# tudelft-iv/CCVPE

Hardware: AMD Instinct MI355X
Metric: image-pairs/sec (higher is better)
Workload: dtype f32

## Files before the change

ccvpe_amd/_lib.py:

```python
import ctypes
import os
import subprocess

import torch

_HERE = os.path.dirname(os.path.abspath(__file__))
LIB_PATH = os.environ.get("CCVPE_LIB") or os.path.join(_HERE, "libccvpe_hip.so")
CSRC_DIR = os.path.join(_HERE, "csrc")

c_float_p = ctypes.c_void_p
c_int = ctypes.c_int
c_float = ctypes.c_float
c_void_p = ctypes.c_void_p


class ConvDesc(ctypes.Structure):
    _fields_ = [
        ("src0", c_void_p), ("src1", c_void_p), ("gate", c_void_p), ("w", c_void_p),
        ("scale", c_void_p), ("shift", c_void_p), ("residual", c_void_p), ("dst", c_void_p),
        ("c0", c_int), ("ld0", c_int), ("c1", c_int), ("ld1", c_int),
        ("batch", c_int), ("in_h", c_int), ("in_w", c_int),
        ("kh", c_int), ("kw", c_int), ("stride", c_int), ("pad", c_int),
        ("n", c_int), ("kpad", c_int), ("ldd", c_int), ("ldres", c_int),
        ("act", c_int), ("out_mode", c_int),
# ... 60 lines not shown
    "ccvpe_upconv3x3_s3_form_ok": (c_int, [ctypes.POINTER(UpconvDesc), c_int]),
    "ccvpe_upconv3x3_s3_route": (c_int, [ctypes.POINTER(UpconvDesc), c_int]),
    "ccvpe_upconv3x3_s3_form_f32": (c_int, [ctypes.POINTER(UpconvDesc), c_int, c_void_p]),
    "ccvpe_set_s3_quad": (c_int, [c_int]),
    "ccvpe_pw_s3_ok": (c_int, [ctypes.POINTER(ConvDesc)]),
    "ccvpe_pw_s3_route": (c_int, [ctypes.POINTER(ConvDesc)]),
    "ccvpe_pw_s3_f32": (c_int, [ctypes.POINTER(ConvDesc), c_void_p]),
    "ccvpe_stem_conv_f32": (c_int, [c_void_p] * 5 + [c_int] * 4 + [c_void_p]),
    "ccvpe_dwconv_nblk": (c_int, [c_int] * 4),
    "ccvpe_dwconv_f32": (c_int, [c_void_p] * 6 + [c_int] * 7 + [c_void_p]),
    "ccvpe_mbconv_front_nblk": (c_int, [c_int] * 6),
    "ccvpe_stem_dw_nblk": (c_int, [c_int] * 3),
    "ccvpe_stem_dw_f32": (c_int, [c_void_p] * 9 + [c_int] * 4 + [c_void_p]),
    "ccvpe_stem_dw_bf16": (c_int, [c_void_p] * 9 + [c_int] * 4 + [c_void_p]),
    "ccvpe_mbconv_front_f32": (c_int, [c_void_p, c_void_p, c_int] + [c_void_p] * 7 + [c_int] * 8 + [c_void_p]),
    "ccvpe_se_gate_f32": (c_int, [c_void_p, c_int, c_float] + [c_void_p] * 5 + [c_int] * 3 + [c_void_p]),
    "ccvpe_ground_descriptor_f32": (c_int, [c_void_p, c_int, c_void_p, c_void_p, ctypes.POINTER(c_int),
                                            c_void_p, c_int, c_int, c_int, c_void_p]),
    "ccvpe_match_level_f32": (c_int, [c_void_p, c_int, c_void_p, c_int, c_int, ctypes.POINTER(c_int),
                                      c_int, c_int, c_int, c_int, c_int, c_void_p, c_void_p, c_int, c_int,
                                      c_int, c_int, c_void_p]),
    "ccvpe_head_conv3x3_f32": (c_int, [c_void_p] * 4 + [c_int] * 5 + [c_void_p]),
    "ccvpe_cast_bf16_f32": (c_int, [c_void_p, c_void_p, ctypes.c_long, c_void_p]),
    "ccvpe_softmax_rows_f32": (c_int, [c_void_p, c_void_p, c_int, c_int, c_void_p]),
    "ccvpe_eval_postprocess_f32": (c_int, [c_void_p, c_void_p, c_void_p, c_int, c_int, c_int, c_void_p]),
    "ccvpe_eval_metrics_f32": (c_int, [c_void_p] * 7 + [c_int, c_int, c_int, c_void_p]),
    "ccvpe_infonce_scratch_floats": (c_int, [c_int, c_int]),
    "ccvpe_infonce_loss_f32": (c_int, [c_void_p, c_void_p, c_float, c_void_p, c_void_p, c_void_p, c_int, c_int, c_void_p]),
    "ccvpe_cross_entropy_loss_f32": (c_int, [c_void_p] * 4 + [c_int, c_int, c_void_p]),
    "ccvpe_orientation_loss_f32": (c_int, [c_void_p] * 5 + [c_int, c_int, c_void_p]),
# ... 132 lines not shown
```

ccvpe_amd/csrc/mbconv_front.hip:

```cpp
#include "common.h"
#include "mbconv_plane.h"
#include <type_traits>

namespace ccvpe {

typedef float f32x4 __attribute__((ext_vector_type(4)));
typedef int mbf_i32x4 __attribute__((ext_vector_type(4)));
__device__ __forceinline__ f32x4 keepv(f32x4 v, bool keep) {
  return __builtin_bit_cast(f32x4, __builtin_bit_cast(mbf_i32x4, v) & (keep ? -1 : 0));
}

struct MbFrontParams {
  const void* x;
  const void* w_exp;
  const float* s0;
  const float* b0;
  const float* w_dw;
  const float* s1;
  const float* b1;
  void* y;
  float* se_partial;
  int H, W, Cin, kpad, mid, Ho, Wo, circular;
  int tiles_x, tiles_y, nchunks, total_blocks;
  int ngroups, cpg;
// ... 157 lines not shown
    for (int o = 4; o < 64; o <<= 1) {
#pragma unroll
      for (int r = 0; r < 4; ++r) sum[r] += __shfl_xor(sum[r], o, 64);
    }
    if (lane < 4) *reinterpret_cast<f32x4*>(red + (wave * 4 + lane) * 4) = sum;
    __syncthreads();
    if (tid < 4) {
      f32x4 t = *reinterpret_cast<const f32x4*>(red + tid * 4);
#pragma unroll
      for (int w = 1; w < 4; ++w) t += *reinterpret_cast<const f32x4*>(red + (w * 4 + tid) * 4);
      *reinterpret_cast<f32x4*>(p.se_partial + ((size_t)b * (p.tiles_x * p.tiles_y) + ty * p.tiles_x + tx) * p.mid + c0 + tid * 4) = t;
    }
  }
}

static int mbf_toh(int k, int stride, int cin) {
  const int n = (cin + 15) / 16;
  if (stride == 2) return n == 1 ? 8 : 4;
  return (n == 1 && k == 3) ? 16 : 8;
}

static bool mbf_supported(int W, int cin, int mid, int k, int sk = 16, int stride = -1) {
  (void)W;
  if (k == 5 && stride == 2 && cin > 32) return false;
  return cin % 8 == 0 && cin <= 16 * MBF_MAX_KK && cin <= sk * MBF_MAX_KK && mid % 16 == 0;
}

}

using namespace ccvpe;
// ... 8 lines not shown
  return ((Ho + toh - 1) / toh) * ((Wo + 15) / 16);
}

extern "C" int ccvpe_mbconv_front_route(int in_h, int in_w, int cin, int mid, int k, int stride, int is_bf16, int batch) {
  if (!(k == 3 || k == 5) || !(stride == 1 || stride == 2)) return CCVPE_EINVAL;
  if (mbf_supported(in_w, cin, mid, k, 16, stride)) return 1;
  if (!(g_mbplane_mode & 1) || mbplane_nblk(in_h, in_w, cin, mid, k, stride) <= 0) return 0;
  return (is_bf16 && (g_mbplane_mode & 4) && mbband_takes(in_h, in_w, cin, mid, k, stride, batch)) ? 3 : 2;
}

extern "C" int ccvpe_mbconv_band_plan(int in_h, int in_w, int cin, int mid, int k, int stride, int batch) {
  if (ccvpe_mbconv_front_route(in_h, in_w, cin, mid, k, stride, 1, batch) != 3) return 0;
  return mbband_plan_packed(in_h, in_w, cin, mid, k, stride, batch);
}

template <typename TE>
static int mbconv_front_any(const void* x, const void* w_exp, int kpad, const float* s0, const float* b0,
                            const float* w_dw, const float* s1, const float* b1, void* y, float* se_partial, int B,
                            int H, int W, int cin, int mid, int k, int stride, int circular, void* stream) {
  constexpr int SK = 4 * (16 / (int)sizeof(TE));
  if (!(k == 3 || k == 5) || !(stride == 1 || stride == 2)) return fail(CCVPE_EINVAL, "mbconv_front: k/stride unsupported");
  if (!mbf_supported(W, cin, mid, k, 16, stride) && (g_mbplane_mode & 1) && mbplane_nblk(H, W, cin, mid, k, stride) > 0)
    return mbplane_launch(sizeof(TE) == 2, 1, x, w_exp, kpad, s0, b0, w_dw, s1, b1, y, se_partial, B, H, W, cin, mid, k, stride,
                          circular, stream);
  if (!mbf_supported(W, cin, mid, k, SK, stride)) return fail(CCVPE_EINVAL, "mbconv_front: shape not supported (W=%d cin=%d mid=%d)", W, cin, mid);
  if (kpad % SK || kpad < cin) return fail(CCVPE_EINVAL, "mbconv_front: bad kpad");
  if (!aligned16(x) || !aligned16(w_exp) || !aligned16(s0) || !aligned16(b0) || !aligned16(s1) || !aligned16(b1) ||
      !aligned16(y) || !aligned16(se_partial) || !aligned16(w_dw))
    return fail(CCVPE_EINVAL, "mbconv_front: pointers must be 16-byte aligned");
  if ((double)H * W * cin * sizeof(TE) >= 4294967296.0) return fail(CCVPE_EINVAL, "mbconv_front: sample larger than 4 GB");
  if (circular && W < k) return fail(CCVPE_EINVAL, "mbconv_front: W too small for circular wrap");
  MbFrontParams p;
  p.x = x; p.w_exp = w_exp; p.s0 = s0; p.b0 = b0; p.w_dw = w_dw; p.s1 = s1; p.b1 = b1; p.y = y; p.se_partial = se_partial;
  p.H = H; p.W = W; p.Cin = cin; p.kpad = kpad; p.mid = mid; p.circular = circular;
  const int total_pad = (stride == 1) ? (k - 1) : (k - 2);
  p.Ho = (H + total_pad - k) / stride + 1;
  p.Wo = (W + total_pad - k) / stride + 1;
  const int toh = mbf_toh(k, stride, cin);
  p.tiles_x = (p.Wo + 15) / 16;
  p.tiles_y = (p.Ho + toh - 1) / toh;
  p.nchunks = mid / 16;
  const long tiles = (long)p.tiles_x * p.tiles_y * B;
  int ng = (int)((2048 + tiles - 1) / tiles);
  if (ng > p.nchunks) ng = p.nchunks;
  if (ng < 1) ng = 1;
  p.cpg = (p.nchunks + ng - 1) / ng;
  p.ngroups = (p.nchunks + p.cpg - 1) / p.cpg;
  const long total = tiles * p.ngroups;
  if (total > 0x7fffffffL) return fail(CCVPE_EINVAL, "mbconv_front: grid too large");
  p.total_blocks = (int)total;
  hipStream_t st = (hipStream_t)stream;
  const int nkk = (cin + SK - 1) / SK;
  int rc = CCVPE_OK;
  auto go = [&](auto kern, int lds_floats) {
    const int lds = lds_floats * 4;
    static DevCache lds_set;
    if ((rc = ensure_dyn_lds(lds_set, kern, lds, "mbconv_front"))) return;
    hipLaunchKernelGGL(kern, dim3(p.total_blocks), dim3(256), lds, st, p);
  };
#define MBF_N(K_, S_, TOH_)                                                                                  \
  if (nkk == 1) go(mbconv_front_kernel<TE, K_, S_, 1, TOH_>, MbfGeom<K_, S_, TOH_>::LDS_FLOATS);                \
  else if (nkk == 2) go(mbconv_front_kernel<TE, K_, S_, 2, TOH_>, MbfGeom<K_, S_, TOH_>::LDS_FLOATS);           \
  else go(mbconv_front_kernel<TE, K_, S_, 3, TOH_>, MbfGeom<K_, S_, TOH_>::LDS_FLOATS)
#define MBF_T(K_, S_, BIG_, SMALL_)                                                                          \
  if (toh == BIG_) { go(mbconv_front_kernel<TE, K_, S_, 1, BIG_>, MbfGeom<K_, S_, BIG_>::LDS_FLOATS); } else { MBF_N(K_, S_, SMALL_); }
// ... 11 lines not shown

extern "C" int ccvpe_mbconv_front_f32(const float* x, const float* w_exp, int kpad, const float* s0, const float* b0,
                                      const float* w_dw, const float* s1, const float* b1, float* y,
                                      float* se_partial, int B, int H, int W, int cin, int mid, int k, int stride,
                                      int circular, void* stream) {
  return mbconv_front_any<float>(x, w_exp, kpad, s0, b0, w_dw, s1, b1, y, se_partial, B, H, W, cin, mid, k, stride,
                                 circular, stream);
}
extern "C" int ccvpe_mbconv_front_bf16(const void* x, const void* w_exp, int kpad, const float* s0, const float* b0,
                                       const float* w_dw, const float* s1, const float* b1, void* y,
                                       float* se_partial, int B, int H, int W, int cin, int mid, int k, int stride,
                                       int circular, void* stream) {
  return mbconv_front_any<cc_bf16>(x, w_exp, kpad, s0, b0, w_dw, s1, b1, y, se_partial, B, H, W, cin, mid, k, stride,
                                   circular, stream);
}
```

ccvpe_amd/csrc/plan.hip:

```cpp
#include <cstring>
#include <string>
#include <unordered_map>
#include <utility>
#include <vector>

#include "common.h"

namespace ccvpe {

enum : uint32_t { K_INT = 0, K_FLT = 1, K_NULL = 2, K_WEIGHTS = 3, K_WORKSPACE = 4, K_GRD = 5, K_SAT = 6, K_STREAM = 7, K_BLOB = 8 };

template <typename A> struct FromSlot {
  static A get(uint64_t v) { return (A)(int64_t)v; }
};
template <typename P> struct FromSlot<P*> {
  static P* get(uint64_t v) { return reinterpret_cast<P*>((uintptr_t)v); }
};
template <> struct FromSlot<float> {
  static float get(uint64_t v) { uint32_t b = (uint32_t)v; float f; std::memcpy(&f, &b, 4); return f; }
};
template <typename... A, size_t... I>
static int invoke_seq(int (*f)(A...), const uint64_t* v, std::index_sequence<I...>) { return f(FromSlot<A>::get(v[I])...); }
template <typename... A>
static int invoke(int (*f)(A...), const uint64_t* v, int n) {
  if (n != (int)sizeof...(A)) return fail(CCVPE_EINVAL, "plan: call has %d arguments, the entry point takes %d", n, (int)sizeof...(A));
  return invoke_seq(f, v, std::index_sequence_for<A...>{});
}
typedef int (*Invoker)(const uint64_t*, int);

#define CCVPE_REG(fn) {#fn, [](const uint64_t* v, int n) -> int { return invoke(fn, v, n); }}
static const std::unordered_map<std::string, Invoker>& registry() {
  static const std::unordered_map<std::string, Invoker> r = {
      CCVPE_REG(ccvpe_conv_igemm_f32), CCVPE_REG(ccvpe_conv_igemm_bf16), CCVPE_REG(ccvpe_conv_igemm_splitk_f32),
      CCVPE_REG(ccvpe_conv_igemm_splitk_bf16), CCVPE_REG(ccvpe_conv3x3_match1_bf16), CCVPE_REG(ccvpe_conv3x3_wino_f32),
      CCVPE_REG(ccvpe_upconv3x3_f32), CCVPE_REG(ccvpe_upconv3x3_bf16), CCVPE_REG(ccvpe_upconv3x3_s3_f32), CCVPE_REG(ccvpe_pw_s3_f32),
      CCVPE_REG(ccvpe_tail512_f32), CCVPE_REG(ccvpe_tail512_bf16), CCVPE_REG(ccvpe_stem_conv_f32), CCVPE_REG(ccvpe_stem_conv_bf16),
      CCVPE_REG(ccvpe_stem_dw_f32), CCVPE_REG(ccvpe_stem_dw_bf16),
      CCVPE_REG(ccvpe_dwconv_f32), CCVPE_REG(ccvpe_dwconv_bf16), CCVPE_REG(ccvpe_mbconv_front_f32), CCVPE_REG(ccvpe_mbconv_front_bf16),
      CCVPE_REG(ccvpe_se_gate_f32), CCVPE_REG(ccvpe_ground_descriptor_f32), CCVPE_REG(ccvpe_match_level_f32),
      CCVPE_REG(ccvpe_match_level_bf16), CCVPE_REG(ccvpe_head_conv3x3_f32), CCVPE_REG(ccvpe_head_conv3x3_bf16),
      CCVPE_REG(ccvpe_softmax_rows_f32), CCVPE_REG(ccvpe_softmax_apply_f32), CCVPE_REG(ccvpe_cast_bf16_f32), CCVPE_REG(ccvpe_eval_postprocess_f32),
  };
  return r;
}
#undef CCVPE_REG

struct Patch { uint32_t call, arg, kind; uint64_t off; };
struct BlobPatch { uint32_t blob, field, kind; uint64_t off; };
struct Call { Invoker fn; std::string name; uint32_t first, nargs, sid; int wait_on; };
struct Output { uint64_t off, bytes; uint32_t dtype, ndim; long long dims[4], strides[4]; };

}

// ... 241 lines not shown
```

ccvpe_amd/models.py:

```python
import torch
import torch.nn as nn

from . import ops
from .synth import B0_BLOCKS, MODEL_SPECS, state_dict_spec

BN_EPS = 1e-3
SKIP_BLOCKS = (15, 10, 4, 2, 0)
MATCH_STRIDES = {"vigor": (64, 32, 16, 8, 4, 2),
                 "kitti": (128, 64, 32, 16, 8, 8),
                 "oxford": (64, 32, 16, 8, 4, 2)}


def window_offset(kind, channels, length):
    return int(channels / 2 - length / 2) if kind == "oxford" else 0


def _round_up(v, m):
    return (v + m - 1) // m * m


class _Holder(nn.Module):

    def forward(self, *a, **k):
        raise RuntimeError("parameter holder is not callable; use the owning CVM_* module")
# ... 59 lines not shown
def _pack_pw_s3(w):
    if w is None or w.dtype != torch.float32 or w.dim() != 2 or w.shape[1] % 16 or w.shape[0] % 16:
        return None
    npad, k = w.shape
    return torch.cat(_split3_bf16(w.reshape(npad, k // 16, 16).permute(1, 0, 2)), -1).contiguous()


def _unpack_pw_s3(w3):
    nst, npad, _ = w3.shape
    return tuple(w3[..., 16 * q:16 * q + 16].float().permute(1, 0, 2).reshape(npad, nst * 16) for q in range(3))


PW_S3_MIN_MID = 240


def _pack_encoder(sd, p, dtype=torch.float32, fold_bn=True, s3=False):
    fold = _fold_bn if fold_bn else (lambda _sd, _p: (None, None))
    e = _Obj()
    e.stem_w = sd[p + "._conv_stem.weight"].permute(2, 3, 1, 0).contiguous()
    e.stem_scale, e.stem_shift = fold(sd, p + "._bn0")
    e.blocks = []
    for i, (k, s, ex, cin, cout) in enumerate(B0_BLOCKS):
        b = _Obj()
        bp = "%s._blocks.%d" % (p, i)
        b.k, b.s, b.expand, b.cin, b.cout, b.mid = k, s, ex != 1, cin, cout, cin * ex
        if b.expand:
            b.w_exp = _pack_conv(sd[bp + "._expand_conv.weight"], dtype)
            b.s0, b.b0 = fold(sd, bp + "._bn0")
        b.w_dw = sd[bp + "._depthwise_conv.weight"].reshape(b.mid, k, k).permute(1, 2, 0).contiguous()
        b.s1, b.b1 = fold(sd, bp + "._bn1")
        b.se_w1 = sd[bp + "._se_reduce.weight"].reshape(-1, b.mid).contiguous()
        b.se_b1 = sd[bp + "._se_reduce.bias"].contiguous()
        b.se_w2 = sd[bp + "._se_expand.weight"].reshape(b.mid, -1).t().contiguous()
        b.se_b2 = sd[bp + "._se_expand.bias"].contiguous()
        b.w_proj = _pack_conv(sd[bp + "._project_conv.weight"], dtype)
        b.w_proj3 = _pack_pw_s3(b.w_proj) if s3 and b.mid >= PW_S3_MIN_MID else None
        b.s2, b.b2 = fold(sd, bp + "._bn2")
        b.skip = (s == 1 and cin == cout)
        e.blocks.append(b)
    e.w_head = _pack_conv(sd[p + "._conv_head.weight"], dtype)
    e.w_head3 = _pack_pw_s3(e.w_head) if s3 else None
    e.head_scale, e.head_shift = fold(sd, p + "._bn1")
    return e
# ... 16 lines not shown
OVERLAP_DECODERS_MAX_BATCH = 128


def _overlap_decoders(precision, batch=1):
    return _OVERLAP_ENV == "1" or (_OVERLAP_ENV == "auto" and precision == "bf16" and batch <= OVERLAP_DECODERS_MAX_BATCH)
FOLD_LEVELS = tuple(int(c) for c in __import__("os").environ.get("CCVPE_FOLD_LEVELS", "012345"))
FOLD_MIN_PIXELS = int(__import__("os").environ.get("CCVPE_FOLD_MIN_PIXELS", "2048"))
FUSE_TAIL = __import__("os").environ.get("CCVPE_FUSE_TAIL", "1") != "0"
SPLIT_TAIL = __import__("os").environ.get("CCVPE_SPLIT_TAIL", "1") != "0"
WINO = __import__("os").environ.get("CCVPE_WINO", "1") != "0"
SPLIT3 = __import__("os").environ.get("CCVPE_SPLIT3", "1") != "0"
SPLIT3_TAIL = SPLIT3 and __import__("os").environ.get("CCVPE_SPLIT3_TAIL", "1") != "0"
SPLIT3_MIN_OK = 2
SPLIT3_PW = SPLIT3 and __import__("os").environ.get("CCVPE_SPLIT3_PW", "1") != "0"
SPLIT3_PW_MIN_OK = 2
PACK_GRAPH = __import__("os").environ.get("CCVPE_PACK_GRAPH", "1") != "0"
PACK_GATHER = __import__("os").environ.get("CCVPE_PACK_GATHER", "1") != "0"
FUSE_MATCH = __import__("os").environ.get("CCVPE_FUSE_MATCH", "1") != "0"
FUSE_STEM = __import__("os").environ.get("CCVPE_FUSE_STEM", "1") != "0"
EVAL_TWO_STREAMS = __import__("os").environ.get("CCVPE_EVAL_TWO_STREAMS", "1") != "0"


def _tail_split(precision, x, cout):
    if x.dtype != torch.float32:
        return 0
    if precision == "bf16":
        return 1 if SPLIT_TAIL and cout == 1 else 0
    return 2 if SPLIT3 and SPLIT3_TAIL else 0


# ... 206 lines not shown

def _run_encoder(e, img, circular, multiscale, dtype=torch.float32):
    blk0 = e.blocks[0]
    stem_fused = (FUSE_STEM and not blk0.expand and blk0.k == 3 and blk0.s == 1 and blk0.mid == 32
                  and ops.stem_dw_supported(img.shape[2], img.shape[3], circular) > 0)
    x = None if stem_fused else ops.stem_conv(img, e.stem_w, e.stem_scale, e.stem_shift, circular, out_dtype=dtype)
    feats = []
    for blk in e.blocks:
        if x is not None:
            b, h, w, _ = x.shape
        if x is None:
            u, part = ops.stem_dw(img, e.stem_w, e.stem_scale, e.stem_shift, blk.w_dw, blk.s1, blk.b1, circular,
                                  out_dtype=dtype)
            b = u.shape[0]
        elif blk.expand and ops.mbconv_front_supported(h, w, blk.cin, blk.mid, blk.k, blk.s):
            u, part = ops.mbconv_front(x, blk.w_exp, blk.s0, blk.b0, blk.w_dw, blk.s1, blk.b1, blk.mid,
                                       blk.k, blk.s, circular)
        else:
            t = x
            if blk.expand:
                t = ops.conv_igemm(x, blk.cin, blk.w_exp, blk.mid, batch=b, in_h=h, in_w=w,
                                   scale=blk.s0, shift=blk.b0, act=ops.ACT_SWISH)
            u, part = ops.dwconv(t, blk.w_dw, blk.s1, blk.b1, blk.k, blk.s, circular)
        ho, wo = u.shape[1], u.shape[2]
        gate = ops.se_gate(part, ho * wo, blk.se_w1, blk.se_b1, blk.se_w2, blk.se_b2)
        x = _pw(u, blk.mid, blk.w_proj, getattr(blk, "w_proj3", None), blk.cout, batch=b, in_h=ho, in_w=wo, gate=gate,
                scale=blk.s2, shift=blk.b2, residual=x if blk.skip else None)
        if multiscale:
            feats.append(x)
    b, h, w, _ = x.shape
    f = _pw(x, 320, e.w_head, getattr(e, "w_head3", None), 1280, batch=b, in_h=h, in_w=w, scale=e.head_scale,
            shift=e.head_shift, act=ops.ACT_SWISH)
# ... 324 lines not shown
```

ccvpe_amd/ops.py:

```python
import ctypes

import torch

from . import _lib
from ._lib import ConvDesc, check

ACT_NONE, ACT_RELU, ACT_SWISH, ACT_RELU_MASK = 0, 1, 2, 3
SPLIT_K_CALLS = 0
SPLIT_K = __import__("os").environ.get("CCVPE_SPLIT_K", "1") == "1"
OUT_NHWC, OUT_DECONV2X = 0, 1

_recorder = None


def set_recorder(rec):
    global _recorder
    _recorder = rec


class LaunchRecorder(object):

    def __init__(self):
        self.items = []

# ... 531 lines not shown
    part = _empty((b, nblk, mid), device=x.device, dtype=torch.float32)
    rec = _recorder
    ev0 = rec.begin() if rec is not None else None
    fn = lib.ccvpe_mbconv_front_f32 if dt == torch.float32 else lib.ccvpe_mbconv_front_bf16
    check(fn(_ptr(x), _ptr(w_exp), w_exp.shape[1], _ptr(s0), _ptr(b0), _ptr(w_dw), _ptr(s1), _ptr(b1), _ptr(y),
             _ptr(part), b, h, wd, cin, mid, k, stride, int(bool(circular)), _stream()), "ccvpe_mbconv_front")
    if rec is not None:
        flops = 2.0 * b * h * wd * cin * mid + 2.0 * b * ho * wo * mid * k * k
        nbytes = (4.0 if dt == torch.float32 else 2.0) * (b * h * wd * cin + b * ho * wo * mid)
        route = lib.ccvpe_mbconv_front_route(h, wd, cin, mid, k, stride, int(dt != torch.float32), b)
        kname = {1: "mbconv_front_kernel", 2: "mbconv_plane_kernel", 3: "mbconv_band_kernel"}.get(route, "mbconv_front_kernel")
        rec.end("%s<%d,%d>" % (kname, k, stride), "in %dx%dx%d mid %d" % (h, wd, cin, mid), flops, nbytes, ev0)
    return y, part


def se_gate(part, hw, w1, b1, w2, b2):
    lib = _lib.load()
    for t, nm in ((part, "part"), (w1, "w1"), (b1, "b1"), (w2, "w2"), (b2, "b2")):
        _chk(t, nm)
    b, nblk, c = part.shape
    cs = w1.shape[0]
    gate = _empty((b, c), device=part.device, dtype=torch.float32)
    check(lib.ccvpe_se_gate_f32(_ptr(part), nblk, 1.0 / float(hw), _ptr(w1), _ptr(b1), _ptr(w2), _ptr(b2),
                                _ptr(gate), b, c, cs, _stream()), "ccvpe_se_gate_f32")
    return gate


def ground_descriptor(y1, wh, bh, cd):
    lib = _lib.load()
    for t, nm in ((y1, "y1"), (wh, "wh"), (bh, "bh")):
# ... 231 lines not shown
```

ccvpe_amd/plan.py:

```python
import ctypes
import struct
import weakref

import torch

from . import _lib, ops

K_INT, K_FLT, K_NULL, K_WEIGHTS, K_WORKSPACE, K_GRD, K_SAT, K_STREAM, K_BLOB = range(9)
ALIGN = 256

LAUNCHES = ("ccvpe_conv_igemm_f32", "ccvpe_conv_igemm_bf16", "ccvpe_conv_igemm_splitk_f32", "ccvpe_conv_igemm_splitk_bf16",
            "ccvpe_conv3x3_match1_bf16", "ccvpe_conv3x3_wino_f32",
            "ccvpe_upconv3x3_f32", "ccvpe_upconv3x3_bf16", "ccvpe_upconv3x3_s3_f32", "ccvpe_pw_s3_f32", "ccvpe_tail512_f32", "ccvpe_tail512_bf16", "ccvpe_stem_conv_f32",
            "ccvpe_stem_conv_bf16", "ccvpe_stem_dw_f32", "ccvpe_stem_dw_bf16", "ccvpe_dwconv_f32", "ccvpe_dwconv_bf16", "ccvpe_mbconv_front_f32", "ccvpe_mbconv_front_bf16",
            "ccvpe_se_gate_f32", "ccvpe_ground_descriptor_f32", "ccvpe_match_level_f32", "ccvpe_match_level_bf16",
            "ccvpe_head_conv3x3_f32", "ccvpe_head_conv3x3_bf16", "ccvpe_softmax_rows_f32", "ccvpe_softmax_apply_f32", "ccvpe_cast_bf16_f32",
            "ccvpe_eval_postprocess_f32")
QUERIES = ("ccvpe_tail512_partials", "ccvpe_conv3x3_match1_ok", "ccvpe_conv3x3_wino_ok", "ccvpe_upconv3x3_s3_ok", "ccvpe_conv_igemm_splitk_floats", "ccvpe_conv_igemm_route", "ccvpe_conv3x3_variant", "ccvpe_upconv3x3_route", "ccvpe_upconv3x3_s3_route", "ccvpe_pw_s3_ok", "ccvpe_pw_s3_route", "ccvpe_dwconv_nblk", "ccvpe_mbconv_front_nblk", "ccvpe_mbconv_front_route", "ccvpe_mbconv_band_plan", "ccvpe_stem_dw_nblk",
           "ccvpe_last_error", "ccvpe_abi_version")


class _Arena(object):

    def __init__(self, size):
        self.size, self.free, self.peak = size, [(0, size)], 0

    def alloc(self, nbytes):
        n = max(ALIGN, (nbytes + ALIGN - 1) // ALIGN * ALIGN)
        for i, (off, sz) in enumerate(self.free):
            if sz >= n:
                if sz == n:
                    del self.free[i]
                else:
# ... 338 lines not shown
```

include/ccvpe_hip.h:

```cpp
#ifndef CCVPE_HIP_H
#define CCVPE_HIP_H

#ifdef __cplusplus
extern "C" {
#endif

#define CCVPE_OK 0
#define CCVPE_EINVAL (-1)
#define CCVPE_ELAUNCH (-2)

#define CCVPE_ACT_NONE 0
#define CCVPE_ACT_RELU 1
#define CCVPE_ACT_SWISH 2
#define CCVPE_ACT_RELU_MASK 3

#define CCVPE_OUT_NHWC 0
#define CCVPE_OUT_DECONV2X 1

#define CCVPE_MAX_SHIFTS 48

const char* ccvpe_last_error(void);
int ccvpe_abi_version(void);

typedef struct ccvpe_conv_desc {
// ... 106 lines not shown
int ccvpe_stem_dw_nblk(int in_h, int in_w, int circular);
int ccvpe_stem_dw_f32(const float* x_nchw, const float* w, const float* s0, const float* b0, const float* w_dw,
                      const float* s1, const float* b1, float* y, float* se_partial, int batch, int in_h,
                      int in_w, int circular, void* stream);
int ccvpe_stem_dw_bf16(const float* x_nchw, const float* w, const float* s0, const float* b0, const float* w_dw,
                       const float* s1, const float* b1, void* y, float* se_partial, int batch, int in_h,
                       int in_w, int circular, void* stream);

int ccvpe_mbconv_front_nblk(int in_h, int in_w, int cin, int mid, int k, int stride);
int ccvpe_mbconv_front_route(int in_h, int in_w, int cin, int mid, int k, int stride, int is_bf16, int batch);
int ccvpe_mbconv_band_plan(int in_h, int in_w, int cin, int mid, int k, int stride, int batch);
int ccvpe_mbconv_front_f32(const float* x, const float* w_exp, int kpad, const float* s0, const float* b0,
                           const float* w_dw, const float* s1, const float* b1, float* y, float* se_partial,
                           int batch, int in_h, int in_w, int cin, int mid, int k, int stride, int circular,
                           void* stream);

int ccvpe_se_gate_f32(const float* se_partial, int nblk, float inv_hw, const float* w1, const float* b1,
                      const float* w2, const float* b2, float* gate, int batch, int channels,
                      int squeezed, void* stream);

int ccvpe_ground_descriptor_f32(const float* y1, int ld, const float* wh, const float* bh, const int* cd,
                                float* out, int batch, int h, int w, void* stream);

int ccvpe_set_match_mfma(int on);
#define CCVPE_MATCH_ROUTE_INTS 10
int ccvpe_match_route(int elem_size, int L, const int* shifts, int n_shifts, int n_max, int n_tail, int stride,
                      int window_offset, int ldx, int ldo, int batch, int hw, int channels, int* out);
int ccvpe_match_level_f32(const float* x, int ldx, const float* g, int ldg, int L, const int* shifts,
                          int n_shifts, int n_max, int n_tail, int stride, int window_offset, float* scores,
                          float* dstx, int ldo, int batch, int hw, int channels, void* stream);
// ... 175 lines not shown
```

Baseline: 2856.

## Add split-bf16 three-plane MFMA path for fused MBConv expand+depthwise front

Adds a new fused MBConv front kernel for f32 inputs. It splits each activation into three bf16 planes and runs the expand 1x1 conv as bf16 MFMA chains against pre-packed three-plane weights, then feeds a depthwise conv, swish and SE partial sums. The aim is to replace the f32 expand GEMM with bf16 matrix-core work while keeping near-f32 accuracy. Weights are double-buffered in LDS across channel chunks, and the path is gated by a per-shape tile-count threshold. In exchange it uses more LDS and registers, and its result can differ slightly from pure f32.

```diff
diff --git a/ccvpe_amd/_lib.py b/ccvpe_amd/_lib.py
--- a/ccvpe_amd/_lib.py
+++ b/ccvpe_amd/_lib.py
@@ -98,6 +98,8 @@
     "ccvpe_stem_dw_f32": (c_int, [c_void_p] * 9 + [c_int] * 4 + [c_void_p]),
     "ccvpe_stem_dw_bf16": (c_int, [c_void_p] * 9 + [c_int] * 4 + [c_void_p]),
     "ccvpe_mbconv_front_f32": (c_int, [c_void_p, c_void_p, c_int] + [c_void_p] * 7 + [c_int] * 8 + [c_void_p]),
+    "ccvpe_mbconv_front_s3_ok": (c_int, [c_int] * 7),
+    "ccvpe_mbconv_front_s3_f32": (c_int, [c_void_p, c_void_p, c_int] + [c_void_p] * 7 + [c_int] * 8 + [c_void_p]),
     "ccvpe_se_gate_f32": (c_int, [c_void_p, c_int, c_float] + [c_void_p] * 5 + [c_int] * 3 + [c_void_p]),
     "ccvpe_ground_descriptor_f32": (c_int, [c_void_p, c_int, c_void_p, c_void_p, ctypes.POINTER(c_int),
                                             c_void_p, c_int, c_int, c_int, c_void_p]),
diff --git a/ccvpe_amd/csrc/mbconv_front.hip b/ccvpe_amd/csrc/mbconv_front.hip
--- a/ccvpe_amd/csrc/mbconv_front.hip
+++ b/ccvpe_amd/csrc/mbconv_front.hip
@@ -1,5 +1,6 @@
 #include "common.h"
 #include "mbconv_plane.h"
+#include "split3_impl.h"
 #include <type_traits>
 
 namespace ccvpe {
@@ -195,6 +196,218 @@
   }
 }
 
+typedef unsigned mbf_u32x4 __attribute__((ext_vector_type(4)));
+
+template <int K, int S, int NKB, int TOH>
+struct Mbf3Geom {
+  using G = MbfGeom<K, S, TOH>;
+  static constexpr int W_DW = NKB * 16 * S3_ROW;
+  static constexpr int W_OFF = G::LDS_FLOATS;
+  static constexpr int LDS_FLOATS = W_OFF + 2 * W_DW;
+};
+
+template <int K, int S, int NKB, int TOH, int WGS>
+__global__ __launch_bounds__(256, WGS) void mbconv_front_s3_kernel(const MbFrontParams p) {
+  using G = MbfGeom<K, S, TOH>;
+  using G3 = Mbf3Geom<K, S, NKB, TOH>;
+  constexpr int PB = (S == 1) ? (K - 1) / 2 : (K - 2) / 2;
+  constexpr int IW = G::IW, NPX = G::NPX, NT = G::NT, TPW = G::TPW, PITCH = G::PITCH;
+  constexpr int KYU = 1;
+  constexpr int W_DW = G3::W_DW, WPIECES = W_DW / 4, WPT = (WPIECES + 255) / 256;
+  extern __shared__ __attribute__((aligned(16))) float sm[];
+  float* tile = sm;
+  float* wdw = sm + NT * 16 * PITCH;
+  float* red = wdw + 2 * K * K * 16;
+  float* wl = sm + G3::W_OFF;
+
+  const int tid = threadIdx.x;
+  const int lane = tid & 63;
+  const int wave = tid >> 6;
+  const int g4 = lane >> 4;
+
+  int lb;
+  {
+    const int q = p.total_blocks / 8, r = p.total_blocks % 8;
+    const int xcd = blockIdx.x % 8, loc = blockIdx.x / 8;
+    lb = (xcd < r ? xcd * (q + 1) : r * (q + 1) + (xcd - r) * q) + loc;
+  }
+  const int grp = lb % p.ngroups;
+  lb /= p.ngroups;
+  const int tx = lb % p.tiles_x;
+  const int ty = (lb / p.tiles_x) % p.tiles_y;
+  const int b = lb / (p.tiles_x * p.tiles_y);
+  const int oy0 = ty * TOH, ox0 = tx * 16;
+  const int iy0 = oy0 * S - PB, ix0 = ox0 * S - PB;
+  const int q4 = g4 * 4;
+
+  f32x4 sc0, sh0, sc1, sh1, wdr, wr[WPT];
+  const int cg = tid & 3;
+  auto load_chunk_params = [&](int chunk) {
+    const int c0 = chunk * 16;
+#pragma unroll
+    for (int j = 0; j < WPT; ++j) {
+      const int idx = tid + 256 * j;
+      if (idx < WPIECES) {
+        const int kb = idx / 96, pc = idx - kb * 96;
+        wr[j] = *reinterpret_cast<const f32x4*>(reinterpret_cast<const float*>(p.w_exp) + ((size_t)kb * p.mid + c0) * S3_ROW + pc * 4);
+      }
+    }
+    sc0 = *reinterpret_cast<const f32x4*>(p.s0 + c0 + q4);
+    sh0 = *reinterpret_cast<const f32x4*>(p.b0 + c0 + q4);
+    sc1 = *reinterpret_cast<const f32x4*>(p.s1 + c0 + cg * 4);
+    sh1 = *reinterpret_cast<const f32x4*>(p.b1 + c0 + cg * 4);
+    const int wi = tid < K * K * 4 ? tid : 0;
+    wdr = *reinterpret_cast<const f32x4*>(p.w_dw + (size_t)(wi >> 2) * p.mid + c0 + (wi & 3) * 4);
+  };
+  auto park_w = [&](int chunk) {
+#pragma unroll
+    for (int j = 0; j < WPT; ++j) {
+      const int idx = tid + 256 * j;
+      if (idx < WPIECES) *reinterpret_cast<f32x4*>(wl + (chunk & 1) * W_DW + idx * 4) = wr[j];
+    }
+  };
+  const int chunk_begin = grp * p.cpg, chunk_end = min(p.nchunks, chunk_begin + p.cpg);
+  load_chunk_params(chunk_begin);
+
+  const float* xb = reinterpret_cast<const float*>(p.x) + (size_t)b * p.H * p.W * p.Cin;
+  mbf_u32x4 xa1[TPW][NKB], xa2[TPW][NKB];
+  unsigned pvalid = 0;
+#pragma unroll
+  for (int i = 0; i < TPW; ++i) {
+    const int q = 16 * (wave + 4 * i) + (lane & 15);
+    const int hy = q / IW, hx = q - hy * IW;
+    const int gy = iy0 + hy;
+    int gx = ix0 + hx;
+    if (p.circular) gx = gx < 0 ? gx + p.W : (gx >= p.W ? gx - p.W : gx);
+    const bool ok = q < NPX && (unsigned)gy < (unsigned)p.H && (unsigned)gx < (unsigned)p.W;
+    pvalid |= ok ? (1u << i) : 0u;
+    const unsigned off = ok ? (unsigned)((gy * p.W + gx) * p.Cin) * 4u : 0u;
+#pragma unroll
+    for (int kb = 0; kb < NKB; ++kb) {
+      const int ch = kb * 16 + (g4 & 1) * 8;
+      const char* src = reinterpret_cast<const char*>(xb) + off + (unsigned)(ch < p.Cin ? ch : 0) * 4u;
+      const f32x4 v0 = *reinterpret_cast<const f32x4*>(src), v1 = *reinterpret_cast<const f32x4*>(src + 16);
+      u32x2 h0, m0, l0, h1, m1, l1;
+      split3(v0, h0, m0, l0);
+      split3(v1, h1, m1, l1);
+      const mbf_u32x4 hi = {h0[0], h0[1], h1[0], h1[1]}, mi = {m0[0], m0[1], m1[0], m1[1]}, lo = {l0[0], l0[1], l1[0], l1[1]};
+      xa1[i][kb] = g4 < 2 ? hi : mi;
+      xa2[i][kb] = g4 < 2 ? lo : hi;
+    }
+  }
+  park_w(chunk_begin);
+  __syncthreads();
+
+  constexpr int NOUT = G::NOUT;
+  constexpr int NCOLS = (NOUT - 1) * S + K;
+  constexpr int XG = 16 / NOUT;
+  const int oxg = (tid >> 2) % XG;
+  const int oyl = (tid >> 2) / XG;
+  const int oy = oy0 + oyl;
+  const int oxl = oxg * NOUT;
+  const bool row_ok = oy < p.Ho;
+  float* yrow = reinterpret_cast<float*>(p.y) + ((size_t)(b * p.Ho + (row_ok ? oy : 0)) * p.Wo) * p.mid;
+  const float* trow = tile + ((oyl * S) * IW + oxl * S) * PITCH + cg * 4;
+  const S3Frag fr(g4);
+
+  for (int chunk = chunk_begin; chunk < chunk_end; ++chunk) {
+    const int c0 = chunk * 16;
+    float* wd = wdw + (chunk & 1) * K * K * 16;
+    if (tid < K * K * 4) *reinterpret_cast<f32x4*>(wd + tid * 4) = wdr;
+    cc_bf16x8 w1[NKB], w2[NKB], w3[NKB];
+    {
+      const float* wrow = wl + (chunk & 1) * W_DW + (lane & 15) * S3_ROW;
+#pragma unroll
+      for (int kb = 0; kb < NKB; ++kb) {
+        w1[kb] = __builtin_bit_cast(cc_bf16x8, *reinterpret_cast<const f32x4*>(wrow + kb * 16 * S3_ROW + fr.w1));
+        w2[kb] = __builtin_bit_cast(cc_bf16x8, *reinterpret_cast<const f32x4*>(wrow + kb * 16 * S3_ROW + fr.w2));
+        w3[kb] = __builtin_bit_cast(cc_bf16x8, *reinterpret_cast<const f32x4*>(wrow + kb * 16 * S3_ROW + fr.w3));
+      }
+    }
+    auto has = [&](int i) { return i < TPW - 1 || wave + 4 * i < NT; };
+    auto chain = [&](int i) {
+      f32x4 acc = {0.f, 0.f, 0.f, 0.f};
+#pragma unroll
+      for (int kb = 0; kb < NKB; ++kb) {
+        const cc_bf16x8 a1 = __builtin_bit_cast(cc_bf16x8, xa1[i][kb]), a2 = __builtin_bit_cast(cc_bf16x8, xa2[i][kb]);
+        acc = __builtin_amdgcn_mfma_f32_16x16x32_bf16(w1[kb], a1, acc, 0, 0, 0);
+        acc = __builtin_amdgcn_mfma_f32_16x16x32_bf16(w2[kb], a1, acc, 0, 0, 0);
+        acc = __builtin_amdgcn_mfma_f32_16x16x32_bf16(w3[kb], a2, acc, 0, 0, 0);
+      }
+      return acc;
+    };
+    auto finish = [&](int i, f32x4 acc) {
+      f32x4 o;
+#pragma unroll
+      for (int r = 0; r < 4; ++r) o[r] = swishf(acc[r] * sc0[r] + sh0[r]);
+      const bool inside = (pvalid >> i) & 1u;
+#pragma unroll
+      for (int r = 0; r < 4; ++r) o[r] = inside ? o[r] : 0.f;
+      *reinterpret_cast<f32x4*>(tile + (16 * (wave + 4 * i) + (lane & 15)) * PITCH + q4) = o;
+    };
+    constexpr int NPAIR = (TPW + 1) / 2;
+    f32x4 pacc[2][2];
+    pacc[0][0] = chain(0);
+    if (1 < TPW && has(1)) pacc[0][1] = chain(1);
+    __builtin_amdgcn_sched_barrier(0);
+#pragma unroll
+    for (int pp = 0; pp < NPAIR; ++pp) {
+      const int n0 = 2 * pp + 2, n1 = 2 * pp + 3;
+      if (n0 < TPW && has(n0)) pacc[(pp + 1) & 1][0] = chain(n0);
+      if (n1 < TPW && has(n1)) pacc[(pp + 1) & 1][1] = chain(n1);
+      if (has(2 * pp)) finish(2 * pp, pacc[pp & 1][0]);
+      if (2 * pp + 1 < TPW && has(2 * pp + 1)) finish(2 * pp + 1, pacc[pp & 1][1]);
+      __builtin_amdgcn_sched_barrier(0);
+    }
+    const f32x4 sc1c = sc1, sh1c = sh1;
+    __syncthreads();
+    const bool more = chunk + 1 < chunk_end;
+    if (more) load_chunk_params(chunk + 1);
+
+    f32x4 acc[NOUT];
+#pragma unroll
+    for (int t = 0; t < NOUT; ++t) acc[t] = (f32x4){0.f, 0.f, 0.f, 0.f};
+#pragma unroll KYU
+    for (int ky = 0; ky < K; ++ky) {
+      f32x4 col[NCOLS];
+#pragma unroll
+      for (int j = 0; j < NCOLS; ++j) col[j] = *reinterpret_cast<const f32x4*>(trow + (ky * IW + j) * PITCH);
+#pragma unroll
+      for (int kx = 0; kx < K; ++kx) {
+        const f32x4 wv = *reinterpret_cast<const f32x4*>(wd + (ky * K + kx) * 16 + cg * 4);
+#pragma unroll
+        for (int t = 0; t < NOUT; ++t) acc[t] += col[t * S + kx] * wv;
+      }
+    }
+    f32x4 sum = {0.f, 0.f, 0.f, 0.f};
+#pragma unroll
+    for (int t = 0; t < NOUT; ++t) {
+      const int ox = ox0 + oxl + t;
+      f32x4 o = acc[t] * sc1c + sh1c;
+#pragma unroll
+      for (int r = 0; r < 4; ++r) o[r] = swishf(o[r]);
+      if (row_ok && ox < p.Wo) {
+        st4<float>(yrow + (size_t)ox * p.mid + c0 + cg * 4, o);
+        sum += o;
+      }
+    }
+#pragma unroll
+    for (int o = 4; o < 64; o <<= 1) {
+#pragma unroll
+      for (int r = 0; r < 4; ++r) sum[r] += __shfl_xor(sum[r], o, 64);
+    }
+    if (lane < 4) *reinterpret_cast<f32x4*>(red + (wave * 4 + lane) * 4) = sum;
+    if (more) park_w(chunk + 1);
+    __syncthreads();
+    if (tid < 4) {
+      f32x4 t = *reinterpret_cast<const f32x4*>(red + tid * 4);
+#pragma unroll
+      for (int w = 1; w < 4; ++w) t += *reinterpret_cast<const f32x4*>(red + (w * 4 + tid) * 4);
+      *reinterpret_cast<f32x4*>(p.se_partial + ((size_t)b * (p.tiles_x * p.tiles_y) + ty * p.tiles_x + tx) * p.mid + c0 + tid * 4) = t;
+    }
+  }
+}
+
 static int mbf_toh(int k, int stride, int cin) {
   const int n = (cin + 15) / 16;
   if (stride == 2) return n == 1 ? 8 : 4;
@@ -233,29 +446,20 @@
   return mbband_plan_packed(in_h, in_w, cin, mid, k, stride, batch);
 }
 
-template <typename TE>
-static int mbconv_front_any(const void* x, const void* w_exp, int kpad, const float* s0, const float* b0,
-                            const float* w_dw, const float* s1, const float* b1, void* y, float* se_partial, int B,
-                            int H, int W, int cin, int mid, int k, int stride, int circular, void* stream) {
-  constexpr int SK = 4 * (16 / (int)sizeof(TE));
-  if (!(k == 3 || k == 5) || !(stride == 1 || stride == 2)) return fail(CCVPE_EINVAL, "mbconv_front: k/stride unsupported");
-  if (!mbf_supported(W, cin, mid, k, 16, stride) && (g_mbplane_mode & 1) && mbplane_nblk(H, W, cin, mid, k, stride) > 0)
-    return mbplane_launch(sizeof(TE) == 2, 1, x, w_exp, kpad, s0, b0, w_dw, s1, b1, y, se_partial, B, H, W, cin, mid, k, stride,
-                          circular, stream);
-  if (!mbf_supported(W, cin, mid, k, SK, stride)) return fail(CCVPE_EINVAL, "mbconv_front: shape not supported (W=%d cin=%d mid=%d)", W, cin, mid);
-  if (kpad % SK || kpad < cin) return fail(CCVPE_EINVAL, "mbconv_front: bad kpad");
+static int mbf_fill(MbFrontParams& p, int& toh, size_t esize, const void* x, const void* w_exp, int kpad, const float* s0, const float* b0,
+                    const float* w_dw, const float* s1, const float* b1, void* y, float* se_partial, int B, int H, int W, int cin,
+                    int mid, int k, int stride, int circular) {
   if (!aligned16(x) || !aligned16(w_exp) || !aligned16(s0) || !aligned16(b0) || !aligned16(s1) || !aligned16(b1) ||
       !aligned16(y) || !aligned16(se_partial) || !aligned16(w_dw))
     return fail(CCVPE_EINVAL, "mbconv_front: pointers must be 16-byte aligned");
-  if ((double)H * W * cin * sizeof(TE) >= 4294967296.0) return fail(CCVPE_EINVAL, "mbconv_front: sample larger than 4 GB");
+  if ((double)H * W * cin * esize >= 4294967296.0) return fail(CCVPE_EINVAL, "mbconv_front: sample larger than 4 GB");
   if (circular && W < k) return fail(CCVPE_EINVAL, "mbconv_front: W too small for circular wrap");
-  MbFrontParams p;
   p.x = x; p.w_exp = w_exp; p.s0 = s0; p.b0 = b0; p.w_dw = w_dw; p.s1 = s1; p.b1 = b1; p.y = y; p.se_partial = se_partial;
   p.H = H; p.W = W; p.Cin = cin; p.kpad = kpad; p.mid = mid; p.circular = circular;
   const int total_pad = (stride == 1) ? (k - 1) : (k - 2);
   p.Ho = (H + total_pad - k) / stride + 1;
   p.Wo = (W + total_pad - k) / stride + 1;
-  const int toh = mbf_toh(k, stride, cin);
+  toh = mbf_toh(k, stride, cin);
   p.tiles_x = (p.Wo + 15) / 16;
   p.tiles_y = (p.Ho + toh - 1) / toh;
   p.nchunks = mid / 16;
@@ -268,6 +472,23 @@
   const long total = tiles * p.ngroups;
   if (total > 0x7fffffffL) return fail(CCVPE_EINVAL, "mbconv_front: grid too large");
   p.total_blocks = (int)total;
+  return CCVPE_OK;
+}
+
+template <typename TE>
+static int mbconv_front_any(const void* x, const void* w_exp, int kpad, const float* s0, const float* b0,
+                            const float* w_dw, const float* s1, const float* b1, void* y, float* se_partial, int B,
+                            int H, int W, int cin, int mid, int k, int stride, int circular, void* stream) {
+  constexpr int SK = 4 * (16 / (int)sizeof(TE));
+  if (!(k == 3 || k == 5) || !(stride == 1 || stride == 2)) return fail(CCVPE_EINVAL, "mbconv_front: k/stride unsupported");
+  if (!mbf_supported(W, cin, mid, k, 16, stride) && (g_mbplane_mode & 1) && mbplane_nblk(H, W, cin, mid, k, stride) > 0)
+    return mbplane_launch(sizeof(TE) == 2, 1, x, w_exp, kpad, s0, b0, w_dw, s1, b1, y, se_partial, B, H, W, cin, mid, k, stride,
+                          circular, stream);
+  if (!mbf_supported(W, cin, mid, k, SK, stride)) return fail(CCVPE_EINVAL, "mbconv_front: shape not supported (W=%d cin=%d mid=%d)", W, cin, mid);
+  if (kpad % SK || kpad < cin) return fail(CCVPE_EINVAL, "mbconv_front: bad kpad");
+  MbFrontParams p;
+  int toh;
+  if (int rc0 = mbf_fill(p, toh, sizeof(TE), x, w_exp, kpad, s0, b0, w_dw, s1, b1, y, se_partial, B, H, W, cin, mid, k, stride, circular)) return rc0;
   hipStream_t st = (hipStream_t)stream;
   const int nkk = (cin + SK - 1) / SK;
   int rc = CCVPE_OK;
@@ -309,3 +530,56 @@
   return mbconv_front_any<cc_bf16>(x, w_exp, kpad, s0, b0, w_dw, s1, b1, y, se_partial, B, H, W, cin, mid, k, stride,
                                    circular, stream);
 }
+
+static bool mbf3_served(int in_w, int cin, int mid, int k, int stride) {
+  if (!(k == 3 || k == 5) || !(stride == 1 || stride == 2) || !mbf_supported(in_w, cin, mid, k, 16, stride)) return false;
+  const int nkb = (cin + 15) / 16;
+  return (k == 3 && stride == 2 && (nkb == 1 || nkb == 3)) || (k == 3 && stride == 1 && nkb == 2) || (k == 5 && stride == 2 && nkb == 2) ||
+         (k == 5 && stride == 1 && nkb == 3);
+}
+
+static bool mbf3_measured(int in_h, int in_w, int cin, int k, int stride, int batch) {
+  const int nkb = (cin + 15) / 16;
+  if (nkb == 1) return false;
+  const int total_pad = (stride == 1) ? (k - 1) : (k - 2);
+  const int Ho = (in_h + total_pad - k) / stride + 1, Wo = (in_w + total_pad - k) / stride + 1;
+  const int toh = mbf_toh(k, stride, cin);
+  const long tiles = (long)batch * ((Ho + toh - 1) / toh) * ((Wo + 15) / 16);
+  if (k == 3 && stride == 1) return tiles >= 1024;
+  if (k == 5 && stride == 2) return tiles >= 3200;
+  if (k == 5 && stride == 1) return tiles >= 1600;
+  return tiles >= 960;
+}
+
+extern "C" int ccvpe_mbconv_front_s3_ok(int in_h, int in_w, int cin, int mid, int k, int stride, int batch) {
+  if (in_h <= 0 || in_w <= 0 || batch <= 0 || !mbf3_served(in_w, cin, mid, k, stride)) return 0;
+  return mbf3_measured(in_h, in_w, cin, k, stride, batch) ? 2 : 1;
+}
+
+extern "C" int ccvpe_mbconv_front_s3_f32(const float* x, const void* w_exp3, int kpad, const float* s0, const float* b0,
+                                         const float* w_dw, const float* s1, const float* b1, float* y, float* se_partial, int B, int H,
+                                         int W, int cin, int mid, int k, int stride, int circular, void* stream) {
+  if (!mbf3_served(W, cin, mid, k, stride)) return fail(CCVPE_EINVAL, "mbconv_front_s3: shape not served (W=%d cin=%d mid=%d k=%d s=%d)", W, cin, mid, k, stride);
+  const int nkb = (cin + 15) / 16;
+  if (kpad != 48 * nkb) return fail(CCVPE_EINVAL, "mbconv_front_s3: kpad %d is not the three-plane pack's (%d)", kpad, 48 * nkb);
+  MbFrontParams p;
+  int toh;
+  if (int rc0 = mbf_fill(p, toh, 4, x, w_exp3, kpad, s0, b0, w_dw, s1, b1, y, se_partial, B, H, W, cin, mid, k, stride, circular)) return rc0;
+  hipStream_t st = (hipStream_t)stream;
+  int rc = CCVPE_OK;
+  auto go = [&](auto kern, int lds_floats) {
+    const int lds = lds_floats * 4;
+    static DevCache lds_set;
+    if ((rc = ensure_dyn_lds(lds_set, kern, lds, "mbconv_front_s3"))) return;
+    hipLaunchKernelGGL(kern, dim3(p.total_blocks), dim3(256), lds, st, p);
+  };
+#define MBF3(K_, S_, NKB_, TOH_, WGS_) if (toh != TOH_) return fail(CCVPE_EINVAL, "mbconv_front_s3: tile height"); else go(mbconv_front_s3_kernel<K_, S_, NKB_, TOH_, WGS_>, Mbf3Geom<K_, S_, NKB_, TOH_>::LDS_FLOATS)
+  if (k == 3 && stride == 2 && nkb == 1) MBF3(3, 2, 1, 8, 2);
+  else if (k == 3 && stride == 1) MBF3(3, 1, 2, 8, 3);
+  else if (k == 5 && stride == 2) MBF3(5, 2, 2, 4, 2);
+  else if (k == 5 && stride == 1) MBF3(5, 1, 3, 8, 2);
+  else MBF3(3, 2, 3, 4, 2);
+#undef MBF3
+  if (rc) return rc;
+  return check_launch("mbconv_front_s3_kernel");
+}
diff --git a/ccvpe_amd/csrc/plan.hip b/ccvpe_amd/csrc/plan.hip
--- a/ccvpe_amd/csrc/plan.hip
+++ b/ccvpe_amd/csrc/plan.hip
@@ -37,6 +37,7 @@
       CCVPE_REG(ccvpe_tail512_f32), CCVPE_REG(ccvpe_tail512_bf16), CCVPE_REG(ccvpe_stem_conv_f32), CCVPE_REG(ccvpe_stem_conv_bf16),
       CCVPE_REG(ccvpe_stem_dw_f32), CCVPE_REG(ccvpe_stem_dw_bf16),
       CCVPE_REG(ccvpe_dwconv_f32), CCVPE_REG(ccvpe_dwconv_bf16), CCVPE_REG(ccvpe_mbconv_front_f32), CCVPE_REG(ccvpe_mbconv_front_bf16),
+      CCVPE_REG(ccvpe_mbconv_front_s3_f32),
       CCVPE_REG(ccvpe_se_gate_f32), CCVPE_REG(ccvpe_ground_descriptor_f32), CCVPE_REG(ccvpe_match_level_f32),
       CCVPE_REG(ccvpe_match_level_bf16), CCVPE_REG(ccvpe_head_conv3x3_f32), CCVPE_REG(ccvpe_head_conv3x3_bf16),
       CCVPE_REG(ccvpe_softmax_rows_f32), CCVPE_REG(ccvpe_softmax_apply_f32), CCVPE_REG(ccvpe_cast_bf16_f32), CCVPE_REG(ccvpe_eval_postprocess_f32),
diff --git a/ccvpe_amd/models.py b/ccvpe_amd/models.py
--- a/ccvpe_amd/models.py
+++ b/ccvpe_amd/models.py
@@ -97,6 +97,9 @@
 PW_S3_MIN_MID = 240
 
 
+MB_S3_MAX_CIN = 48
+
+
 def _pack_encoder(sd, p, dtype=torch.float32, fold_bn=True, s3=False):
     fold = _fold_bn if fold_bn else (lambda _sd, _p: (None, None))
     e = _Obj()
@@ -110,6 +113,7 @@
         if b.expand:
             b.w_exp = _pack_conv(sd[bp + "._expand_conv.weight"], dtype)
             b.s0, b.b0 = fold(sd, bp + "._bn0")
+            b.w_exp3 = _pack_pw_s3(b.w_exp) if s3 and cin <= MB_S3_MAX_CIN else None
         b.w_dw = sd[bp + "._depthwise_conv.weight"].reshape(b.mid, k, k).permute(1, 2, 0).contiguous()
         b.s1, b.b1 = fold(sd, bp + "._bn1")
         b.se_w1 = sd[bp + "._se_reduce.weight"].reshape(-1, b.mid).contiguous()
@@ -156,6 +160,8 @@
 SPLIT3_MIN_OK = 2
 SPLIT3_PW = SPLIT3 and __import__("os").environ.get("CCVPE_SPLIT3_PW", "1") != "0"
 SPLIT3_PW_MIN_OK = 2
+SPLIT3_MB = SPLIT3 and __import__("os").environ.get("CCVPE_SPLIT3_MB", "1") != "0"
+SPLIT3_MB_MIN_OK = 2
 PACK_GRAPH = __import__("os").environ.get("CCVPE_PACK_GRAPH", "1") != "0"
 PACK_GATHER = __import__("os").environ.get("CCVPE_PACK_GATHER", "1") != "0"
 FUSE_MATCH = __import__("os").environ.get("CCVPE_FUSE_MATCH", "1") != "0"
@@ -392,8 +398,12 @@
                                   out_dtype=dtype)
             b = u.shape[0]
         elif blk.expand and ops.mbconv_front_supported(h, w, blk.cin, blk.mid, blk.k, blk.s):
-            u, part = ops.mbconv_front(x, blk.w_exp, blk.s0, blk.b0, blk.w_dw, blk.s1, blk.b1, blk.mid,
-                                       blk.k, blk.s, circular)
+            w3 = getattr(blk, "w_exp3", None)
+            if SPLIT3 and SPLIT3_MB and w3 is not None and ops.mbconv_front_s3_ok(x, w3, blk.mid, blk.k, blk.s) >= SPLIT3_MB_MIN_OK:
+                u, part = ops.mbconv_front_s3(x, w3, blk.s0, blk.b0, blk.w_dw, blk.s1, blk.b1, blk.mid, blk.k, blk.s, circular)
+            else:
+                u, part = ops.mbconv_front(x, blk.w_exp, blk.s0, blk.b0, blk.w_dw, blk.s1, blk.b1, blk.mid,
+                                           blk.k, blk.s, circular)
         else:
             t = x
             if blk.expand:
diff --git a/ccvpe_amd/ops.py b/ccvpe_amd/ops.py
--- a/ccvpe_amd/ops.py
+++ b/ccvpe_amd/ops.py
@@ -569,6 +569,43 @@
     return y, part
 
 
+def mbconv_front_s3_ok(x, w_exp3, mid, k, stride):
+    if w_exp3 is None or x.dtype != torch.float32 or w_exp3.dtype != torch.bfloat16:
+        return 0
+    b, h, wd, cin = x.shape
+    if w_exp3.dim() != 3 or tuple(w_exp3.shape) != ((cin + 15) // 16, mid, 48):
+        return 0
+    return int(_lib.load().ccvpe_mbconv_front_s3_ok(h, wd, cin, mid, k, stride, b))
+
+
+def mbconv_front_s3(x, w_exp3, s0, b0, w_dw, s1, b1, mid, k, stride, circular):
+    lib = _lib.load()
+    _chk(x, "x", torch.float32)
+    _chk(w_exp3, "w_exp3", torch.bfloat16)
+    for t, nm in ((s0, "s0"), (b0, "b0"), (w_dw, "w_dw"), (s1, "s1"), (b1, "b1")):
+        _chk(t, nm)
+    b, h, wd, cin = x.shape
+    if w_exp3.dim() != 3 or tuple(w_exp3.shape) != ((cin + 15) // 16, mid, 48):
+        raise ValueError("w_exp3 is not the three-plane pack of models._pack_pw_s3 for cin = %d, mid = %d" % (cin, mid))
+    nblk = mbconv_front_supported(h, wd, cin, mid, k, stride)
+    if nblk == 0 or not lib.ccvpe_mbconv_front_s3_ok(h, wd, cin, mid, k, stride, b):
+        raise _lib.CcvpeError("mbconv_front_s3: unsupported shape %s k=%d stride=%d" % (tuple(x.shape), k, stride))
+    tot = (k - 1) if stride == 1 else (k - 2)
+    ho, wo = (h + tot - k) // stride + 1, (wd + tot - k) // stride + 1
+    y = _empty((b, ho, wo, mid), device=x.device, dtype=torch.float32)
+    part = _empty((b, nblk, mid), device=x.device, dtype=torch.float32)
+    rec = _recorder
+    ev0 = rec.begin() if rec is not None else None
+    check(lib.ccvpe_mbconv_front_s3_f32(_ptr(x), _ptr(w_exp3), w_exp3.shape[0] * w_exp3.shape[2], _ptr(s0), _ptr(b0), _ptr(w_dw),
+                                        _ptr(s1), _ptr(b1), _ptr(y), _ptr(part), b, h, wd, cin, mid, k, stride,
+                                        int(bool(circular)), _stream()), "ccvpe_mbconv_front_s3_f32")
+    if rec is not None:
+        flops = 2.0 * b * h * wd * cin * mid + 2.0 * b * ho * wo * mid * k * k
+        nbytes = 4.0 * (b * h * wd * cin + b * ho * wo * mid)
+        rec.end("mbconv_front_s3_kernel<%d,%d>" % (k, stride), "in %dx%dx%d mid %d" % (h, wd, cin, mid), flops, nbytes, ev0)
+    return y, part
+
+
 def se_gate(part, hw, w1, b1, w2, b2):
     lib = _lib.load()
     for t, nm in ((part, "part"), (w1, "w1"), (b1, "b1"), (w2, "w2"), (b2, "b2")):
diff --git a/ccvpe_amd/plan.py b/ccvpe_amd/plan.py
--- a/ccvpe_amd/plan.py
+++ b/ccvpe_amd/plan.py
@@ -12,11 +12,11 @@
 LAUNCHES = ("ccvpe_conv_igemm_f32", "ccvpe_conv_igemm_bf16", "ccvpe_conv_igemm_splitk_f32", "ccvpe_conv_igemm_splitk_bf16",
             "ccvpe_conv3x3_match1_bf16", "ccvpe_conv3x3_wino_f32",
             "ccvpe_upconv3x3_f32", "ccvpe_upconv3x3_bf16", "ccvpe_upconv3x3_s3_f32", "ccvpe_pw_s3_f32", "ccvpe_tail512_f32", "ccvpe_tail512_bf16", "ccvpe_stem_conv_f32",
-            "ccvpe_stem_conv_bf16", "ccvpe_stem_dw_f32", "ccvpe_stem_dw_bf16", "ccvpe_dwconv_f32", "ccvpe_dwconv_bf16", "ccvpe_mbconv_front_f32", "ccvpe_mbconv_front_bf16",
+            "ccvpe_stem_conv_bf16", "ccvpe_stem_dw_f32", "ccvpe_stem_dw_bf16", "ccvpe_dwconv_f32", "ccvpe_dwconv_bf16", "ccvpe_mbconv_front_f32", "ccvpe_mbconv_front_bf16", "ccvpe_mbconv_front_s3_f32",
             "ccvpe_se_gate_f32", "ccvpe_ground_descriptor_f32", "ccvpe_match_level_f32", "ccvpe_match_level_bf16",
             "ccvpe_head_conv3x3_f32", "ccvpe_head_conv3x3_bf16", "ccvpe_softmax_rows_f32", "ccvpe_softmax_apply_f32", "ccvpe_cast_bf16_f32",
             "ccvpe_eval_postprocess_f32")
-QUERIES = ("ccvpe_tail512_partials", "ccvpe_conv3x3_match1_ok", "ccvpe_conv3x3_wino_ok", "ccvpe_upconv3x3_s3_ok", "ccvpe_conv_igemm_splitk_floats", "ccvpe_conv_igemm_route", "ccvpe_conv3x3_variant", "ccvpe_upconv3x3_route", "ccvpe_upconv3x3_s3_route", "ccvpe_pw_s3_ok", "ccvpe_pw_s3_route", "ccvpe_dwconv_nblk", "ccvpe_mbconv_front_nblk", "ccvpe_mbconv_front_route", "ccvpe_mbconv_band_plan", "ccvpe_stem_dw_nblk",
+QUERIES = ("ccvpe_tail512_partials", "ccvpe_conv3x3_match1_ok", "ccvpe_conv3x3_wino_ok", "ccvpe_upconv3x3_s3_ok", "ccvpe_conv_igemm_splitk_floats", "ccvpe_conv_igemm_route", "ccvpe_conv3x3_variant", "ccvpe_upconv3x3_route", "ccvpe_upconv3x3_s3_route", "ccvpe_pw_s3_ok", "ccvpe_pw_s3_route", "ccvpe_dwconv_nblk", "ccvpe_mbconv_front_nblk", "ccvpe_mbconv_front_route", "ccvpe_mbconv_front_s3_ok", "ccvpe_mbconv_band_plan", "ccvpe_stem_dw_nblk",
            "ccvpe_last_error", "ccvpe_abi_version")
 
 
diff --git a/include/ccvpe_hip.h b/include/ccvpe_hip.h
--- a/include/ccvpe_hip.h
+++ b/include/ccvpe_hip.h
@@ -144,6 +144,11 @@
                            const float* w_dw, const float* s1, const float* b1, float* y, float* se_partial,
                            int batch, int in_h, int in_w, int cin, int mid, int k, int stride, int circular,
                            void* stream);
+int ccvpe_mbconv_front_s3_ok(int in_h, int in_w, int cin, int mid, int k, int stride, int batch);
+int ccvpe_mbconv_front_s3_f32(const float* x, const void* w_exp3, int kpad, const float* s0, const float* b0,
+                              const float* w_dw, const float* s1, const float* b1, float* y, float* se_partial,
+                              int batch, int in_h, int in_w, int cin, int mid, int k, int stride, int circular,
+                              void* stream);
 
 int ccvpe_se_gate_f32(const float* se_partial, int nblk, float inv_hw, const float* w1, const float* b1,
                       const float* w2, const float* b2, float* gate, int batch, int channels,
```

Result: faster. 2886, median of 6 (+1.1%).
